# ChanTsune/Portable-Network-Archive

Hardware: AMD Instinct MI355X
Metric: archive-create MiB/s (input bytes/sec), zstd-3, 10000 x 1 MiB enwik-style corpus (higher is better)
Workload: dtype u8

## Files before the change

portable-network-archive_amd/csrc/k_lz_split.hip:

```cpp
#include <type_traits>
#include "lz_common.h"

namespace pna {


#define DPP_ROW_SHL1(v) ((uint32_t)__builtin_amdgcn_update_dpp(0, (int)(v), 0x101, 0xF, 0xF, true))
constexpr uint32_t PK_LEN = 26, PK_OFF = 6, PK_LOW = (1u << PK_LEN) - 1;
__host__ __device__ constexpr uint32_t pkb_of(int strong) { return strong == 2 ? 2u : 3u; }
__device__ __forceinline__ uint32_t pk_make(uint32_t l, uint32_t off, uint32_t bkf) { return (l << PK_LEN) | ((off << PK_OFF) | bkf); }
template <uint32_t S, uint32_t PKB = 3>
__device__ __forceinline__ uint32_t pk_adopt(uint32_t P, uint32_t Pn) {
    constexpr uint32_t BM = PKB == 2 ? 0x3Cu : 0x38u;
    const uint32_t T = Pn + ((S << PK_LEN) - (S << PKB));
    const bool a = (Pn & (BM & ~((S - 1) << PKB))) != 0 && T > (P | PK_LOW);
    return a ? T : P;
}
#define DPP_ROW_SHL2(v) ((uint32_t)__builtin_amdgcn_update_dpp(0, (int)(v), 0x102, 0xF, 0xF, true))
__device__ __forceinline__ uint32_t ffbh_hw(uint32_t x) { uint32_t r; asm("v_ffbh_u32 %0, %1" : "=v"(r) : "v"(x)); return r; }
__device__ __forceinline__ uint32_t back15_field(uint32_t x1, uint32_t x2, uint32_t x3, uint32_t x4) {
    const uint32_t f1 = ffbh_hw(x1), f2 = __builtin_elementwise_add_sat(ffbh_hw(x2), 32u), f3 = __builtin_elementwise_add_sat(ffbh_hw(x3), 64u), f4 = ffbh_hw(x4 | 0xFFu) + 96u;
    uint32_t n, m;
    asm("v_min3_u32 %0, %1, %2, %3" : "=v"(n) : "v"(f2), "v"(f3), "v"(f4));
    asm("v_min_u32 %0, %1, %2" : "=v"(m) : "v"(f1), "v"(n));
    return (m >> 1) & 0x3Cu;
// ... 391 lines not shown
                    l = 16 + first_diff16(y0, y1, y2, y3);
                }
                if (edge) { const uint32_t lim = blk_end - q; l = l < lim ? l : lim; }
                const uint32_t bqj = j ? __builtin_amdgcn_alignbyte(D[0], Dm1, j) : Dm1;
                const uint32_t xk = bqj ^ bc;
                uint32_t bk3 = (uint32_t)__builtin_clz(xk | 0xFFu) & 24u;
                if (STRONG == 1 && xk == 0) { const uint32_t bq2 = j ? __builtin_amdgcn_alignbyte(Dm1, Dm2, j) : Dm2; bk3 = 32u + ((uint32_t)__builtin_clz((bq2 ^ bc2) | 0xFFu) & 24u); }
                if (STRONG == 2) {
                    lds_cu32 *pe = lds_word(WB8 + 8 + ((c8 - 8) & ~3u));
                    const uint32_t e0 = pe[0], e1 = pe[1], p0 = pc[0];
                    const uint32_t bq2 = j ? __builtin_amdgcn_alignbyte(Dm1, Dm2, j) : Dm2, bq3 = j ? __builtin_amdgcn_alignbyte(Dm2, Dm3, j) : Dm3, bq4 = j ? __builtin_amdgcn_alignbyte(Dm3, Dm4, j) : Dm4;
                    bk3 = back15_field(xk, bq2 ^ bc2, bq3 ^ __builtin_amdgcn_alignbit(p0, e1, shc), bq4 ^ __builtin_amdgcn_alignbit(e1, e0, shc));
                }
                Pj = STRONG ? (l >= MIN_MATCH ? pk_make(l, o, bk3) : 0u) : pk_make(l >= MIN_MATCH ? l : 0u, o, bk3);
            }
            P[j] = Pj;
        }
        if (adopt) {
            if (STRONG == 2) {
                uint32_t P8[4];
#pragma unroll
                for (int j = 0; j < 4; j++) P8[j] = DPP_ROW_SHL2(P[j]);
#pragma unroll
                for (int j = 0; j < 4; j++) P[j] = pk_adopt<8, PKB>(P[j], P8[j]);
            }
            if (STRONG) {
                uint32_t P4[4];
#pragma unroll
                for (int j = 0; j < 4; j++) P4[j] = DPP_ROW_SHL1(P[j]);
#pragma unroll
                for (int j = 0; j < 4; j++) P[j] = pk_adopt<4, PKB>(P[j], P4[j]);
            }
            {
                const uint32_t Pn = DPP_ROW_SHL1(P[0]);
                const uint32_t P1[4] = {P[1], P[2], P[3], Pn};
#pragma unroll
                for (int j = 0; j < 4; j++) P[j] = pk_adopt<1, PKB>(P[j], P1[j]);
            }
            {
                const uint32_t Pa = DPP_ROW_SHL1(P[0]), Pb = DPP_ROW_SHL1(P[1]);
                const uint32_t P2[4] = {P[2], P[3], Pa, Pb};
#pragma unroll
                for (int j = 0; j < 4; j++) P[j] = pk_adopt<2, PKB>(P[j], P2[j]);
            }
        }
        if (q0 < t1) {
            if (W3) {
                uint32_t ww[4];
#pragma unroll
                for (int j = 0; j < 4; j++) {
                    const uint32_t l = P[j] >> PK_LEN, lc = l < 5u ? 5u : (l > 36u ? 36u : l);
                    ww[j] = (lc - 5u) | ((P[j] >> (PK_OFF - 5)) & (0xFFFFFu << 5));
                }
                W12 *o = (W12 *)(pb8 + 3 * (size_t)q0);
                __builtin_nontemporal_store(__builtin_amdgcn_perm(ww[1], ww[0], 0x04020100u), &o->x);
                __builtin_nontemporal_store(__builtin_amdgcn_perm(ww[2], ww[1], 0x05040201u), &o->y);
                __builtin_nontemporal_store(__builtin_amdgcn_perm(ww[3], ww[2], 0x06050402u), &o->z);
            } else {
                const uint32_t lmax = (flags & FLAG_LEN36) ? 36u : 63u;
                uint32_t l4[4];
#pragma unroll
                for (int j = 0; j < 4; j++) { const uint32_t l = P[j] >> PK_LEN; l4[j] = l < lmax ? l : lmax; }
                v4u wv;
                wv.x = l4[0] | (P[0] & (0xFFFFFu << PK_OFF)); wv.y = l4[1] | (P[1] & (0xFFFFFu << PK_OFF));
                wv.z = l4[2] | (P[2] & (0xFFFFFu << PK_OFF)); wv.w = l4[3] | (P[3] & (0xFFFFFu << PK_OFF));
                __builtin_nontemporal_store(wv, (v4u *)(pb + q0));
            }
        }
#undef QW
#pragma unroll
        for (int j = 0; j < 4; j++) if (hv[j] && (ins_all || !(j & 1))) atomicMax(&table[hsh[j]], ((q0 + j + 1) << TAG_BITS) | tag[j]);
        __syncthreads();
    }
}

constexpr uint32_t LZP_THREADS = 64;
template <bool CT, int LZD, bool W3>
__global__ __launch_bounds__(LZP_THREADS) __attribute__((amdgpu_waves_per_eu(5, 5)))
void k_lzp(const uint8_t *__restrict__ src, const SegDesc *__restrict__ segs, const uint32_t *__restrict__ blk_seg, uint64_t *__restrict__ seqs, uint8_t *__restrict__ lits,
           BlkInfo *__restrict__ blk, uint4 *__restrict__ ctab, uint32_t flags, uint32_t max_len, const uint32_t *__restrict__ pbuf, uint32_t blk0, uint32_t *__restrict__ hist) {
    constexpr uint32_t RW = 256, TG = 4096;
    static_assert(LZ_G_ZSTD == 4 && LZ_G_DEFLATE == 4 && (1u << BLK_LOG_MIN) % TG == 0 && CAP1 == 32, "k_lzp: regions of 4 groups, tiles of 16 regions");
    __shared__ __attribute__((aligned(16))) uint32_t l32[TG / 4];
    __shared__ uint4 lmask[TG / 64];
    __shared__ uint32_t plut[16];
    uint4 (*rec)[TG / 64] = (uint4 (*)[TG / 64])l32;
    __shared__ uint16_t xlen[16 * 8];
    __shared__ uint32_t shist[192];
    __shared__ uint8_t s_llc[64], s_mlc[128];
    __shared__ uint32_t lstage[264];
    const uint32_t lane = threadIdx.x, w = lane & 15;
    const uint8_t *len8 = (const uint8_t *)l32;
    const uint32_t gb = blk0 + blockIdx.x;
    const SegDesc sd = segs[blk_seg[gb]];
    const uint32_t seg_len = sd.len;
    if ((flags & FLAG_SMALL_ONLY) && seg_len > MID_SEG) return;
    const uint8_t *seg = src + sd.src_off;
    const uint32_t blk_log = sd.blk_log, bsz = 1u << blk_log, SC = seq_cap_of(blk_log);
    const uint32_t *pb = pbuf + ((size_t)(sd.blk_base - blk0) << blk_log);
    const uint8_t *pb8 = (const uint8_t *)pbuf + 3 * ((size_t)(sd.blk_base - blk0) << blk_log);
    auto word_at = [&](uint32_t pos) -> uint32_t {
        if (!W3) return pb[pos];
        const uint32_t x = *(const u32u *)(pb8 + 3 * (size_t)pos) & 0xFFFFFFu, e = x & 31u;
        return (e ? e + 5u : 0u) | ((x >> 5) << 6);
    };
    const uint32_t lazy = flags & F_LAZY;
    const uint32_t wbase = w * RW;
    const uint32_t bs0 = (gb - sd.blk_base) << blk_log, bs1 = seg_len - bs0 < bsz ? seg_len : bs0 + bsz;
    const uint32_t tile0 = bs0 / TG, ntile = bs0 < seg_len ? (bs1 + TG - 1) / TG : tile0;
    const bool lv = lane < 16;
    if (hist) {
        const uint32_t i = lane, m0 = lane, m1 = lane + 64;
        s_llc[i] = (uint8_t)(i < 16 ? i : (i < 24 ? 16 + ((i - 16) >> 1) : (i < 32 ? 20 + ((i - 24) >> 2) : (i < 48 ? 22 + ((i - 32) >> 3) : 24))));
        s_mlc[m0] = (uint8_t)(m0 < 32 ? m0 : (m0 < 40 ? 32 + ((m0 - 32) >> 1) : (m0 < 48 ? 36 + ((m0 - 40) >> 2) : 38 + ((m0 - 48) >> 3))));
        s_mlc[m1] = (uint8_t)(m1 < 96 ? 40 + ((m1 - 64) >> 4) : 42);
    }
    if (lv) {
        uint32_t sel = 0, j = 0;
        for (uint32_t bit = 0; bit < 4; bit++) if ((lane >> bit) & 1) { sel |= bit << (8 * j); j++; }
        plut[lane] = sel;
    }
    const uint64_t lit_below = ((uint64_t)1 << (4 * (lane & 15))) - 1;
    uint32_t next_free = 0, seq_run = 0, lit_run = 0, g_last1 = 1;
    uint32_t lcarry = 0;

    for (uint32_t T = tile0; T < ntile; T++) {
        const uint32_t t0 = T * TG, blk_start = t0 & ~(bsz - 1);
        const uint32_t blk_end = (seg_len - blk_start < bsz) ? seg_len : blk_start + bsz;
        const uint32_t t1 = (blk_end - t0 < TG) ? blk_end : t0 + TG;
        const uint32_t npos = t1 - t0;
        const uint32_t ext_lim = (t1 + LOOKAHEAD < blk_end) ? t1 + LOOKAHEAD : blk_end;
        const uint32_t gblk = sd.blk_base + (t0 >> blk_log);
        const uint32_t ng = (npos + 63) >> 6;
        {
            const uint4 *pt = (const uint4 *)(pb + t0);
            const W12 *pt3 = (const W12 *)(pb8 + 3 * (size_t)t0);
            for (uint32_t wq = 0; wq < 4 && wq * 1024 < npos; wq++) {
                uint4 v[4]; W12 v3[4];
#pragma unroll
                for (uint32_t i = 0; i < 4; i++) { if (W3) v3[i] = pt3[(wq * 4 + i) * 64 + lane]; else v[i] = pt[(wq * 4 + i) * 64 + lane]; }
#pragma unroll
                for (uint32_t i = 0; i < 4; i++) {
                    const uint32_t p = (wq * 4 + i) * RW + lane * 4;
                    uint32_t d;
                    if (W3) {
                        const uint32_t E = (v3[i].x & 31u) | (((v3[i].x >> 24) & 31u) << 8) | (((v3[i].y >> 16) & 31u) << 16) | (((v3[i].z >> 8) & 31u) << 24);
                        const uint32_t nz = ((E + 0x1F1F1F1Fu) >> 5) & 0x01010101u;
                        d = E + nz * 5u;
                    } else d = (v[i].x & 63u) | ((v[i].y & 63u) << 8) | ((v[i].z & 63u) << 16) | ((v[i].w & 63u) << 24);
                    if (npos < TG && p + 4 > npos) d = p >= npos ? 0u : d & (0xFFFFFFFFu >> (8 * (p + 4 - npos)));
                    l32[p >> 2] = d;
                }
            }
        }
        __builtin_amdgcn_wave_barrier();
        if (lane < ng) {
            uint32_t d[17];
#pragma unroll
            for (uint32_t i = 0; i < 4; i++) { const uint4 t = ((const uint4 *)l32)[lane * 4 + i]; d[4 * i] = t.x; d[4 * i + 1] = t.y; d[4 * i + 2] = t.z; d[4 * i + 3] = t.w; }
            d[16] = 0;
            uint32_t em2[2] = {0, 0}, cm2[2] = {0, 0};
#pragma unroll
            for (uint32_t i = 0; i < 16; i++) {
                const uint32_t x = d[i] | 0x80808080u;
                uint32_t e = x - 0x06060606u;
                if (lazy) {
                    e &= x - __builtin_amdgcn_alignbyte(d[i + 1], d[i], 1);
                    if (LZD >= 2) e &= x + 0x01010101u - __builtin_amdgcn_alignbyte(d[i + 1], d[i], 2);
                    if (LZD >= 3) e &= x + 0x02020202u - __builtin_amdgcn_alignbyte(d[i + 1], d[i], 3);
                }
                const uint32_t en = ((((e >> 7) & 0x01010101u) * 0x00204081u) >> 21) & 15u;
                const uint32_t cn = ((((d[i] >> 5) & 0x01010101u) * 0x00204081u) >> 21) & 15u;
                em2[i >> 3] |= en << (4 * (i & 7)); cm2[i >> 3] |= cn << (4 * (i & 7));
            }
            lmask[lane] = make_uint4(em2[0], em2[1], cm2[0], cm2[1]);
        }
        __builtin_amdgcn_wave_barrier();
        if (t0 == blk_start) { next_free = blk_start; seq_run = 0; lit_run = 0; g_last1 = 1; lcarry = 0;
                               if (hist) { for (uint32_t i = lane; i < 192; i += 64) shist[i] = 0; __builtin_amdgcn_wave_barrier(); } }
        const uint32_t c_in = next_free > t0 ? next_free - t0 : 0u;
        uint64_t sel[4], cov[4], cm[4];
        uint32_t el = 0, nx = 0;
        uint32_t em_lo[4], em_hi[4], cm_lo[4], cm_hi[4];
#pragma unroll
        for (int r = 0; r < 4; r++) {
            uint4 m = make_uint4(0, 0, 0, 0);
            if (lv && w * 4 + r < ng) m = lmask[w * 4 + r];
            em_lo[r] = m.x; em_hi[r] = m.y; cm_lo[r] = m.z; cm_hi[r] = m.w;
        }
        {
            uint32_t cur = c_in > wbase ? (c_in - wbase < RW ? c_in - wbase : RW) : 0u;
            uint32_t s32[8], c32[8];
#pragma unroll
            for (int hb = 0; hb < 8; hb++) {
                const uint32_t em32 = (hb & 1) ? em_hi[hb >> 1] : em_lo[hb >> 1], cm32 = (hb & 1) ? cm_hi[hb >> 1] : cm_lo[hb >> 1];
                const uint32_t e0 = cur > 32u * hb ? cur - 32u * hb : 0u;
                uint32_t rem = e0 < 32 ? em32 & (0xFFFFFFFFu << e0) : 0u;
                uint32_t e_last = e0, selr = 0, covr = e0 < 32 ? (1u << e0) - 1 : 0xFFFFFFFFu;
                while (__ballot(rem != 0)) {
                    const bool a = rem != 0;
                    const uint32_t s = a ? (uint32_t)__builtin_ctz(rem) : 0u;
                    const uint32_t ps = wbase + 32u * hb + s;
                    uint32_t L = a ? len8[ps] : 0u;
                    const bool cap = a && ((cm32 >> s) & 1);
                    uint64_t need = __ballot(cap);
                    if (need) {
                        const uint32_t qs = t0 + ps;
                        const uint32_t pwv = cap ? word_at(qs) : 0u;
                        const uint32_t xl = ext_lim - qs < max_len ? ext_lim - qs : max_len;
                        while (need) {
                            const uint32_t k = ctz64(need); need &= need - 1;
                            const uint32_t qk = rdlane(qs, k), ok = rdlane(pwv >> 6, k);
                            const uint32_t Lk = lz_extend_mem(seg, seg_len, qk, qk - ok, rdlane(L, k), rdlane(xl, k), lane);
                            if (lane == k) L = Lk;
                        }
                        if (cap) { xlen[w * 8 + (nx & 7)] = (uint16_t)L; nx++; }
                    }
                    if (a) {
                        const uint32_t e = s + L;
                        const uint32_t me = e < 32 ? (1u << e) - 1 : 0xFFFFFFFFu;
                        selr |= 1u << s; e_last = e;
                        covr |= me & ~((1u << s) - 1);
                        rem &= ~me;
                    }
                }
                s32[hb] = selr; c32[hb] = covr;
                if (selr) el = 32u * hb + e_last;
                cur = 32u * hb + (e_last > 32 ? e_last : 32u);
            }
#pragma unroll
            for (int r = 0; r < 4; r++) {
                sel[r] = (uint64_t)s32[2 * r] | ((uint64_t)s32[2 * r + 1] << 32); cov[r] = (uint64_t)c32[2 * r] | ((uint64_t)c32[2 * r + 1] << 32);
                cm[r] = (uint64_t)cm_lo[r] | ((uint64_t)cm_hi[r] << 32);
            }
        }
        uint32_t pc[4];
        pc[0] = 0;
#pragma unroll
        for (int r = 0; r < 3; r++) pc[r + 1] = pc[r] + (uint32_t)__popcll(sel[r] & cm[r]);

        uint32_t E = c_in, tile_exit;
        {
            const uint32_t wend = el ? wbase + el : 0u;
            uint32_t x = c_in;
#pragma unroll
            for (uint32_t k = 0; k < 16; k++) {
                const uint32_t ek = rdlane(wend, k);
                if (w == k) E = x;
                if (x < k * RW + RW && ek >= x + CUT_MIN) x = ek;
            }
            tile_exit = x;
        }
        uint64_t fsel[4], litm[4];
        uint32_t nselp[5], nlitp[5];
        uint32_t cut_r = 4, cut_b = 0, cut_len = 0, cut_off = 0;
        {
            const uint32_t Ew = E > wbase ? (E - wbase < RW ? E - wbase : RW) : 0u;
            const uint32_t in0 = t1 > t0 + wbase ? t1 - (t0 + wbase) : 0u;
            uint64_t K[4], cv[4];
#pragma unroll
            for (int r = 0; r < 4; r++) {
                const uint32_t e = Ew > 64u * r ? Ew - 64u * r : 0u;
                K[r] = mlow(e < 64 ? e : 64u); fsel[r] = sel[r] & ~K[r]; cv[r] = cov[r];
            }
            if (lv && Ew > 0 && Ew < RW) {
                const uint32_t grp = Ew >> 6, b = Ew & 63;
                uint64_t cg = cov[0], sg = sel[0];
#pragma unroll
                for (int r = 1; r < 4; r++) if (grp == (uint32_t)r) { cg = cov[r]; sg = sel[r]; }
                if (((cg >> b) & 1) && !((sg >> b) & 1)) {
                    uint64_t below = sg & mlow(b);
                    uint32_t g2 = grp;
#pragma unroll
                    for (int r = 2; r >= 0; r--) if (!below && (uint32_t)r < grp && sel[r]) { below = sel[r]; g2 = (uint32_t)r; }
                    const uint32_t s2 = 63 - clz64(below);
                    const uint32_t pw2 = word_at(t0 + wbase + 64 * g2 + s2);
                    uint64_t sc2 = sel[0] & cm[0]; uint32_t pc2 = pc[0];
#pragma unroll
                    for (int r = 1; r < 4; r++) if (g2 == (uint32_t)r) { sc2 = sel[r] & cm[r]; pc2 = pc[r]; }
                    const uint32_t l2 = ((sc2 >> s2) & 1) ? xlen[w * 8 + ((pc2 + (uint32_t)__popcll(sc2 & mlow(s2))) & 7)] : (pw2 & 63u);
                    const uint32_t end2 = 64 * g2 + s2 + l2, rmn = end2 - Ew;
                    if (rmn >= CUT_MIN) {
#pragma unroll
                        for (int r = 0; r < 4; r++) if (grp == (uint32_t)r) fsel[r] |= (uint64_t)1 << b;
                        cut_r = grp; cut_b = b; cut_len = rmn; cut_off = pw2 >> 6;
                    } else {
                        uint32_t fx_s = RW, fx_x = 0;
                        if (end2 < RW) {
                            uint64_t eg = 0, eg1 = 0, cg2 = 0, cg3 = 0;
#pragma unroll
                            for (int r = 0; r < 4; r++) {
                                const uint64_t e64 = (uint64_t)em_lo[r] | ((uint64_t)em_hi[r] << 32);
                                if (grp == (uint32_t)r) { eg = e64; cg2 = cm[r]; }
                                if (grp + 1 == (uint32_t)r) { eg1 = e64; cg3 = cm[r]; }
                            }
                            const uint32_t want = (1u << rmn) - 1u;
                            const uint32_t w8 = (uint32_t)((eg >> b) | (b ? eg1 << (64 - b) : 0)) & want, c8 = (uint32_t)((cg2 >> b) | (b ? cg3 << (64 - b) : 0));
                            if (w8) {
                                const uint32_t ds = (uint32_t)__builtin_ctz(w8), sp = Ew + ds;
                                const uint32_t L = len8[wbase + sp], x = sp + L;
                                if (!((c8 >> ds) & 1) && x < RW && x < in0) {
                                    const uint32_t gx = x >> 6, bx = x & 63;
                                    uint64_t cvx = cov[0], slx = sel[0];
#pragma unroll
                                    for (int r = 1; r < 4; r++) if (gx == (uint32_t)r) { cvx = cov[r]; slx = sel[r]; }
                                    if (!((cvx >> bx) & 1) || ((slx >> bx) & 1)) { fx_s = sp; fx_x = x; }
                                }
                            }
                        }
#pragma unroll
                        for (int r = 0; r < 4; r++) {
                            const uint32_t a0 = Ew > 64u * r ? (Ew - 64u * r < 64 ? Ew - 64u * r : 64u) : 0u;
                            const uint32_t zend = fx_s < RW ? fx_x : end2;
                            const uint32_t z0 = zend > 64u * r ? (zend - 64u * r < 64 ? zend - 64u * r : 64u) : 0u;
                            cv[r] &= ~(mlow(z0) & ~mlow(a0));
                            if (fx_s < RW) {
                                const uint32_t s0 = fx_s > 64u * r ? (fx_s - 64u * r < 64 ? fx_s - 64u * r : 64u) : 0u;
                                cv[r] |= mlow(z0) & ~mlow(s0);
                                fsel[r] &= ~mlow(z0);
                                if ((fx_s >> 6) == (uint32_t)r) fsel[r] |= (uint64_t)1 << (fx_s & 63);
                            }
                        }
                    }
                }
            }
            nselp[0] = 0; nlitp[0] = 0;
#pragma unroll
            for (int r = 0; r < 4; r++) {
                const uint32_t ir = in0 > 64u * r ? in0 - 64u * r : 0u;
                litm[r] = lv ? mlow(ir < 64 ? ir : 64u) & ~(cv[r] | K[r]) : 0;
                if (!lv) fsel[r] = 0;
                nselp[r + 1] = nselp[r] + (uint32_t)__popcll(fsel[r]);
                nlitp[r + 1] = nlitp[r] + (uint32_t)__popcll(litm[r]);
            }
        }
        uint32_t gl = 0, gf = 0;
#pragma unroll
        for (int r = 3; r >= 0; r--) if (!gl && fsel[r]) { const uint32_t sp = 63 - clz64(fsel[r]); gl = 1 + nlitp[r] + (uint32_t)__popcll(litm[r] & mlow(sp)); }
        if (CT) {
#pragma unroll
            for (int r = 0; r < 4; r++) if (!gf && fsel[r]) { const uint32_t sp = ctz64(fsel[r]); gf = 1 + nlitp[r] + (uint32_t)__popcll(litm[r] & mlow(sp)); }
        }
        {
            const uint32_t cnt = nselp[4] | (nlitp[4] << 16);
            const uint32_t incl = row_scan_add(cnt), excl = incl - cnt;
            const uint32_t gabs = gl ? lit_run + (excl >> 16) + gl : 0u;
            const uint32_t gmax = row_scan_max(gabs);
            const uint32_t tot = rdlane(incl, 15);
            const uint32_t seq_base = seq_run + (excl & 0xFFFF), lit_base = lit_run + (excl >> 16);
            const uint32_t gb = DPP_ROW_SHR(gmax, 1);
            const uint32_t glast1_before = gb > g_last1 ? gb : g_last1;
            const uint32_t ga = rdlane(gmax, 15);
            if (CT) {
                constexpr uint32_t CH = TG / TILE, WPC = 16 / CH;
                const uint32_t hrow = (uint32_t)__ballot(gl != 0) & 0xFFFFu;
#pragma unroll
                for (uint32_t h = 0; h < CH; h++) {
                    const uint32_t ex_h = rdlane(excl, h * WPC);
                    const uint32_t hm_h = hrow & (((1u << WPC) - 1) << (h * WPC));
                    uint32_t g_first = lit_run + (tot >> 16);
                    if (hm_h) { const uint32_t j0 = (uint32_t)__builtin_ctz(hm_h); g_first = lit_run + (rdlane(excl, j0) >> 16) + rdlane(gf, j0) - 1; }
                    if (lane == 0) ctab[((size_t)gblk << (blk_log - 11)) + (t0 - blk_start) / TILE + h] = make_uint4(seq_run + (ex_h & 0xFFFF), lit_run + (ex_h >> 16), g_first, 0u);
                }
            }
            g_last1 = ga > g_last1 ? ga : g_last1;
            seq_run += tot & 0xFFFF; lit_run += tot >> 16;
            next_free = t0 + rdlane(tile_exit, 0);
            asm volatile("" ::: "memory");
            if (lv) {
                uint32_t prevl = 0; bool any = false;
#pragma unroll
                for (int r = 0; r < 4; r++) {
                    const uint32_t llbase = any ? nlitp[r] - prevl : lit_base + nlitp[r] - (glast1_before - 1);
                    if (fsel[r]) { const uint32_t sp = 63 - clz64(fsel[r]); prevl = nlitp[r] + (uint32_t)__popcll(litm[r] & mlow(sp)); any = true; }
                    const uint64_t sc = sel[r] & cm[r];
                    const uint32_t cutw = cut_r == (uint32_t)r ? cut_b | (cut_len << 8) : 64u;
                    rec[0][w * 4 + r] = make_uint4((uint32_t)litm[r], (uint32_t)(litm[r] >> 32), lit_base + nlitp[r], seq_base + nselp[r]);
                    rec[1][w * 4 + r] = make_uint4((uint32_t)fsel[r], (uint32_t)(fsel[r] >> 32), (uint32_t)sc, (uint32_t)(sc >> 32));
                    rec[2][w * 4 + r] = make_uint4(llbase, w * 8 + pc[r], cutw, cut_off);
                }
            }
            if (t1 == blk_end && lane == 0) { blk[gblk].nseq = seq_run; blk[gblk].nlit = lit_run; }
        }
        __builtin_amdgcn_wave_barrier();
        uint32_t lw[16];
        if (t0 + TG <= seg_len) {
#pragma unroll
            for (uint32_t wr = 0; wr < 16; wr++) lw[wr] = *(const uint32_t *)(seg + t0 + wr * RW + 4 * lane);
        } else {
#pragma unroll
            for (uint32_t wr = 0; wr < 16; wr++) {
                const uint32_t q = t0 + wr * RW + 4 * lane;
                lw[wr] = 0;
                if (q + 4 <= seg_len) lw[wr] = *(const uint32_t *)(seg + q);
                else { for (uint32_t i = 0; i < 3; i++) if (q + i < seg_len) lw[wr] |= (uint32_t)seg[q + i] << (8 * i); }
            }
        }
        {
            uint64_t *bseq = seqs + (size_t)gblk * SC;
            const uint4 ra = rec[0][lane], rb = rec[1][lane], rc = rec[2][lane];
            const uint64_t lm = (uint64_t)ra.x | ((uint64_t)ra.y << 32), sc = (uint64_t)rb.z | ((uint64_t)rb.w << 32);
            uint64_t rem = lane < ng ? (uint64_t)rb.x | ((uint64_t)rb.y << 32) : 0;
            uint32_t idx = ra.w, prev = 0;
            const uint32_t cut_b2 = rc.z & 0xFFu, cut_l2 = rc.z >> 8;
            bool first = true;
            const uint32_t pg0 = t0 + lane * 64;
            while (rem) {
                uint32_t sq[4], pw[4];
#pragma unroll
                for (int u = 0; u < 4; u++) {
                    sq[u] = rem ? ctz64(rem) : 64u;
                    pw[u] = rem ? word_at(pg0 + sq[u]) : 0u;
                    rem &= rem - 1;
                }
#pragma unroll
                for (int u = 0; u < 4; u++) {
                    const uint32_t s = sq[u];
                    if (s < 64) {
                        uint32_t ml = pw[u] & 63u, of = pw[u] >> 6;
                        if ((sc >> s) & 1) ml = xlen[(rc.y + (uint32_t)__popcll(sc & mlow(s))) & 127];
                        if (cut_b2 == s) { ml = cut_l2; of = rc.w; }
                        const uint32_t lq = (uint32_t)__popcll(lm & mlow(s));
                        const uint32_t ll = first ? rc.x + lq : lq - prev;
                        if (idx < SC) bseq[idx] = seq_pack(ll, ml, of);
                        if (hist) {
                            const uint32_t mb = ml - 3u, of3 = of + 3u;
                            uint32_t *hh = shist;
                            atomicAdd(&hh[ll < 64 ? (uint32_t)s_llc[ll] : 50u - (uint32_t)__builtin_clz(ll)], 1u);
                            atomicAdd(&hh[64 + 31u - (uint32_t)__builtin_clz(of3)], 1u);
                            atomicAdd(&hh[128 + (mb < 128 ? (uint32_t)s_mlc[mb] : 67u - (uint32_t)__builtin_clz(mb))], 1u);
                        }
                        idx++; prev = lq; first = false;
                    }
                }
            }
        }
        if (hist && t1 == blk_end) {
            __builtin_amdgcn_wave_barrier(); asm volatile("" ::: "memory");
            uint32_t *hs = hist + (size_t)blk_seg[gb] * 448u + 256u;
            for (uint32_t i = lane; i < 192; i += 64) { const uint32_t v = shist[i]; if (v) atomicAdd(&hs[i], v); }
        }
        {
            uint8_t *blit = lits + ((size_t)gblk << blk_log);
            const uint32_t sh = 4 * (lane & 15);
            uint8_t *stage8 = (uint8_t *)lstage;
#pragma unroll
            for (uint32_t wq = 0; wq < 4; wq++) {
                if (wq * 1024 >= npos) continue;
                const uint32_t L0 = rec[0][wq * 16].z, L1 = wq < 3 ? rec[0][wq * 16 + 16].z : lit_run;
                const uint32_t A0 = L0 & ~3u;
                if (lane == 0) lstage[0] = lcarry;
                __builtin_amdgcn_wave_barrier(); asm volatile("" ::: "memory");
#pragma unroll
                for (uint32_t i = 0; i < 4; i++) {
                    const uint32_t wr = wq * 4 + i;
                    if (wr * RW >= npos) continue;
                    const uint4 m = rec[0][wr * 4 + (lane >> 4)];
                    const uint32_t wd = lw[wr];
                    const uint64_t lm = (uint64_t)m.x | ((uint64_t)m.y << 32);
                    const uint32_t nib = (uint32_t)(lm >> sh) & 15u;
                    const uint32_t pk = __builtin_amdgcn_perm(wd, wd, plut[nib]), cnt = (uint32_t)__popc(nib);
                    uint8_t *o = stage8 + (m.z + (uint32_t)__popcll(lm & lit_below) - A0);
                    if (cnt > 0) o[0] = (uint8_t)pk;
                    if (cnt > 1) o[1] = (uint8_t)(pk >> 8);
                    if (cnt > 2) o[2] = (uint8_t)(pk >> 16);
                    if (cnt > 3) o[3] = (uint8_t)(pk >> 24);
                }
                __builtin_amdgcn_wave_barrier(); asm volatile("" ::: "memory");
                const uint32_t nfull = (L1 - A0) >> 2;
                uint32_t *g32 = (uint32_t *)(blit + A0);
                for (uint32_t j = lane; j < nfull; j += 64) g32[j] = lstage[j];
                lcarry = uni(lstage[nfull]);
                __builtin_amdgcn_wave_barrier(); asm volatile("" ::: "memory");
            }
            if (t1 == blk_end) {
                const uint32_t rem = lit_run & 3u;
                if (lane < rem) blit[(lit_run & ~3u) + lane] = (uint8_t)(lcarry >> (8 * lane));
            }
        }
        __builtin_amdgcn_wave_barrier();
        asm volatile("" ::: "memory");
    }
}

template <bool CT, int STRONG, uint32_t GLOG, uint32_t WLOG, bool FARP = !CT, bool TAB3 = false>
static void launch_split_g(const uint8_t *src, const SegDesc *segs, uint32_t nseg, uint64_t *seqs, uint8_t *lits, BlkInfo *blk, uint4 *ctab,
                           uint32_t flags, uint32_t max_off, uint32_t max_len, hipStream_t st, uint32_t *pbuf, uint32_t blk0, hipEvent_t ev_match, uint32_t *gtab, const LzParseGrid *pg) {
    constexpr uint32_t LT = GLOG ? LzGeo<WLOG>::L_TABLE : LzGeo<WLOG, TAB3>::L_TOTAL;
    static const hipError_t attr_set = hipFuncSetAttribute((const void *)k_lzm<CT, STRONG, GLOG, WLOG, FARP, TAB3>, hipFuncAttributeMaxDynamicSharedMemorySize, (int)LzGeo<WLOG, TAB3>::L_TOTAL);
    (void)attr_set;
    constexpr bool W3 = GLOG == 0;
    if (!(flags & FLAG_ALL_SMALL)) hipLaunchKernelGGL((k_lzm<CT, STRONG, GLOG, WLOG, FARP, TAB3>), dim3(nseg), dim3(LZ_THREADS), LT, st, src, segs, flags, max_off, pbuf, blk0, gtab);
    if (flags & FLAG_TIER1) hipLaunchKernelGGL((k_lzms<STRONG, W3>), dim3(nseg), dim3(64), lzms_lds(SMALL_SEG), st, src, segs, flags, pbuf, blk0, 0u, SMALL_SEG);
    if (flags & FLAG_TIER2) { const uint32_t mx = 8192u + 4096u * ((flags >> FLAG_T2_SHIFT) & 3u);
                              hipLaunchKernelGGL((k_lzms<STRONG, W3>), dim3(nseg), dim3(64), lzms_lds(mx), st, src, segs, flags, pbuf, blk0, SMALL_SEG, mx); }
    if (ev_match) (void)hipEventRecord(ev_match, st);
    if (!pg || pg->nb == 0) return;
    if (flags & FLAG_LAZY3) hipLaunchKernelGGL((k_lzp<CT, 3, W3>), dim3(pg->nb), dim3(LZP_THREADS), 0, st, src, pg->segs_all, pg->blk_seg, seqs, lits, blk, ctab, flags, max_len, pbuf, blk0, pg->hist);
    else if (flags & FLAG_LAZY2) hipLaunchKernelGGL((k_lzp<CT, 2, W3>), dim3(pg->nb), dim3(LZP_THREADS), 0, st, src, pg->segs_all, pg->blk_seg, seqs, lits, blk, ctab, flags, max_len, pbuf, blk0, pg->hist);
    else hipLaunchKernelGGL((k_lzp<CT, 1, W3>), dim3(pg->nb), dim3(LZP_THREADS), 0, st, src, pg->segs_all, pg->blk_seg, seqs, lits, blk, ctab, flags, max_len, pbuf, blk0, pg->hist);
}
void launch_lz_split(const uint8_t *src, const SegDesc *segs, uint32_t nseg, uint64_t *seqs, uint8_t *lits, BlkInfo *blk, uint4 *ctab,
                     uint32_t flags, uint32_t max_off, uint32_t max_len, hipStream_t st, uint32_t *pbuf, uint32_t blk0, hipEvent_t ev_match, uint32_t *gtab, const LzParseGrid *pg) {
// ... 48 lines not shown
```

Baseline: 145,600.

## Parallelize greedy match selection across all 64 lanes with speculative group resync

The greedy parse over each 256-byte region is no longer walked serially by 16 lanes across four 64-bit groups. All 64 lanes now walk one 64-position group each in parallel, starting at the group boundary, then repair speculation by re-walking from the predecessor's actual end until the walk synchronizes with an already selected match. Extended lengths are packed per lane into two 16-bit slots instead of a shared ring, and prefix scans are widened to span 64 lanes. This is meant to remove the serial dependency and idle lanes in match selection, at the cost of redundant re-walks when groups don't resynchronize. It also caps extended matches at two per group.

Measured after the change: 146,200, median of 6. About the same (+0.4%).

```diff
diff --git a/portable-network-archive_amd/csrc/k_lz_split.hip b/portable-network-archive_amd/csrc/k_lz_split.hip
--- a/portable-network-archive_amd/csrc/k_lz_split.hip
+++ b/portable-network-archive_amd/csrc/k_lz_split.hip
@@ -497,14 +497,14 @@
     constexpr uint32_t RW = 256, TG = 4096;
     static_assert(LZ_G_ZSTD == 4 && LZ_G_DEFLATE == 4 && (1u << BLK_LOG_MIN) % TG == 0 && CAP1 == 32, "k_lzp: regions of 4 groups, tiles of 16 regions");
     __shared__ __attribute__((aligned(16))) uint32_t l32[TG / 4];
-    __shared__ uint4 lmask[TG / 64];
+    __shared__ uint4 gsc[TG / 64];
     __shared__ uint32_t plut[16];
     uint4 (*rec)[TG / 64] = (uint4 (*)[TG / 64])l32;
-    __shared__ uint16_t xlen[16 * 8];
+    __shared__ uint32_t xlen[TG / 64];
     __shared__ uint32_t shist[192];
     __shared__ uint8_t s_llc[64], s_mlc[128];
     __shared__ uint32_t lstage[264];
-    const uint32_t lane = threadIdx.x, w = lane & 15;
+    const uint32_t lane = threadIdx.x, w = lane >> 2, rq = lane & 3;
     const uint8_t *len8 = (const uint8_t *)l32;
     const uint32_t gb = blk0 + blockIdx.x;
     const SegDesc sd = segs[blk_seg[gb]];
@@ -520,17 +520,16 @@
         return (e ? e + 5u : 0u) | ((x >> 5) << 6);
     };
     const uint32_t lazy = flags & F_LAZY;
-    const uint32_t wbase = w * RW;
+    const uint32_t wbase = w * RW, gb64 = 64 * rq, gbase = 64 * lane;
     const uint32_t bs0 = (gb - sd.blk_base) << blk_log, bs1 = seg_len - bs0 < bsz ? seg_len : bs0 + bsz;
     const uint32_t tile0 = bs0 / TG, ntile = bs0 < seg_len ? (bs1 + TG - 1) / TG : tile0;
-    const bool lv = lane < 16;
     if (hist) {
         const uint32_t i = lane, m0 = lane, m1 = lane + 64;
         s_llc[i] = (uint8_t)(i < 16 ? i : (i < 24 ? 16 + ((i - 16) >> 1) : (i < 32 ? 20 + ((i - 24) >> 2) : (i < 48 ? 22 + ((i - 32) >> 3) : 24))));
         s_mlc[m0] = (uint8_t)(m0 < 32 ? m0 : (m0 < 40 ? 32 + ((m0 - 32) >> 1) : (m0 < 48 ? 36 + ((m0 - 40) >> 2) : 38 + ((m0 - 48) >> 3))));
         s_mlc[m1] = (uint8_t)(m1 < 96 ? 40 + ((m1 - 64) >> 4) : 42);
     }
-    if (lv) {
+    if (lane < 16) {
         uint32_t sel = 0, j = 0;
         for (uint32_t bit = 0; bit < 4; bit++) if ((lane >> bit) & 1) { sel |= bit << (8 * j); j++; }
         plut[lane] = sel;
@@ -569,6 +568,7 @@
             }
         }
         __builtin_amdgcn_wave_barrier();
+        uint64_t em = 0, cm = 0;
         if (lane < ng) {
             uint32_t d[17];
 #pragma unroll
@@ -588,193 +588,192 @@
                 const uint32_t cn = ((((d[i] >> 5) & 0x01010101u) * 0x00204081u) >> 21) & 15u;
                 em2[i >> 3] |= en << (4 * (i & 7)); cm2[i >> 3] |= cn << (4 * (i & 7));
             }
-            lmask[lane] = make_uint4(em2[0], em2[1], cm2[0], cm2[1]);
-        }
-        __builtin_amdgcn_wave_barrier();
+            em = (uint64_t)em2[0] | ((uint64_t)em2[1] << 32); cm = (uint64_t)cm2[0] | ((uint64_t)cm2[1] << 32);
+        }
         if (t0 == blk_start) { next_free = blk_start; seq_run = 0; lit_run = 0; g_last1 = 1; lcarry = 0;
                                if (hist) { for (uint32_t i = lane; i < 192; i += 64) shist[i] = 0; __builtin_amdgcn_wave_barrier(); } }
         const uint32_t c_in = next_free > t0 ? next_free - t0 : 0u;
-        uint64_t sel[4], cov[4], cm[4];
-        uint32_t el = 0, nx = 0;
-        uint32_t em_lo[4], em_hi[4], cm_lo[4], cm_hi[4];
-#pragma unroll
-        for (int r = 0; r < 4; r++) {
-            uint4 m = make_uint4(0, 0, 0, 0);
-            if (lv && w * 4 + r < ng) m = lmask[w * 4 + r];
-            em_lo[r] = m.x; em_hi[r] = m.y; cm_lo[r] = m.z; cm_hi[r] = m.w;
-        }
+        const uint32_t rent = c_in > wbase ? (c_in - wbase < RW ? c_in - wbase : RW) : 0u;
+        uint64_t sel = 0, cov;
+        uint32_t ext, le = 0, xl2 = 0;
+        auto walk_len = [&](bool a, uint32_t s) -> uint32_t {
+            uint32_t L = a ? len8[gbase + s] : 0u;
+            const bool cap = a && ((cm >> s) & 1);
+            uint64_t need = __ballot(cap);
+            if (need) {
+                const uint32_t qs = t0 + gbase + s;
+                const uint32_t pwv = cap ? word_at(qs) : 0u;
+                const uint32_t xl = ext_lim - qs < max_len ? ext_lim - qs : max_len;
+                while (need) {
+                    const uint32_t k = ctz64(need); need &= need - 1;
+                    const uint32_t qk = rdlane(qs, k), ok = rdlane(pwv >> 6, k);
+                    const uint32_t Lk = lz_extend_mem(seg, seg_len, qk, qk - ok, rdlane(L, k), rdlane(xl, k), lane);
+                    if (lane == k) L = Lk;
+                }
+            }
+            return L;
+        };
+        const uint32_t ent = rent > gb64 ? rent : gb64;
         {
-            uint32_t cur = c_in > wbase ? (c_in - wbase < RW ? c_in - wbase : RW) : 0u;
-            uint32_t s32[8], c32[8];
-#pragma unroll
-            for (int hb = 0; hb < 8; hb++) {
-                const uint32_t em32 = (hb & 1) ? em_hi[hb >> 1] : em_lo[hb >> 1], cm32 = (hb & 1) ? cm_hi[hb >> 1] : cm_lo[hb >> 1];
-                const uint32_t e0 = cur > 32u * hb ? cur - 32u * hb : 0u;
-                uint32_t rem = e0 < 32 ? em32 & (0xFFFFFFFFu << e0) : 0u;
-                uint32_t e_last = e0, selr = 0, covr = e0 < 32 ? (1u << e0) - 1 : 0xFFFFFFFFu;
-                while (__ballot(rem != 0)) {
-                    const bool a = rem != 0;
-                    const uint32_t s = a ? (uint32_t)__builtin_ctz(rem) : 0u;
-                    const uint32_t ps = wbase + 32u * hb + s;
-                    uint32_t L = a ? len8[ps] : 0u;
-                    const bool cap = a && ((cm32 >> s) & 1);
-                    uint64_t need = __ballot(cap);
-                    if (need) {
-                        const uint32_t qs = t0 + ps;
-                        const uint32_t pwv = cap ? word_at(qs) : 0u;
-                        const uint32_t xl = ext_lim - qs < max_len ? ext_lim - qs : max_len;
-                        while (need) {
-                            const uint32_t k = ctz64(need); need &= need - 1;
-                            const uint32_t qk = rdlane(qs, k), ok = rdlane(pwv >> 6, k);
-                            const uint32_t Lk = lz_extend_mem(seg, seg_len, qk, qk - ok, rdlane(L, k), rdlane(xl, k), lane);
-                            if (lane == k) L = Lk;
-                        }
-                        if (cap) { xlen[w * 8 + (nx & 7)] = (uint16_t)L; nx++; }
-                    }
-                    if (a) {
-                        const uint32_t e = s + L;
-                        const uint32_t me = e < 32 ? (1u << e) - 1 : 0xFFFFFFFFu;
-                        selr |= 1u << s; e_last = e;
-                        covr |= me & ~((1u << s) - 1);
-                        rem &= ~me;
-                    }
-                }
-                s32[hb] = selr; c32[hb] = covr;
-                if (selr) el = 32u * hb + e_last;
-                cur = 32u * hb + (e_last > 32 ? e_last : 32u);
-            }
-#pragma unroll
-            for (int r = 0; r < 4; r++) {
-                sel[r] = (uint64_t)s32[2 * r] | ((uint64_t)s32[2 * r + 1] << 32); cov[r] = (uint64_t)c32[2 * r] | ((uint64_t)c32[2 * r + 1] << 32);
-                cm[r] = (uint64_t)cm_lo[r] | ((uint64_t)cm_hi[r] << 32);
-            }
-        }
-        uint32_t pc[4];
-        pc[0] = 0;
-#pragma unroll
-        for (int r = 0; r < 3; r++) pc[r + 1] = pc[r] + (uint32_t)__popcll(sel[r] & cm[r]);
+            const uint32_t e0 = ent - gb64;
+            cov = mlow(e0);
+            uint64_t rem = em & ~cov;
+            uint32_t nx = 0;
+            while (__ballot(rem != 0)) {
+                const bool a = rem != 0;
+                const uint32_t s = a ? ctz64(rem) : 0u;
+                const uint32_t L = walk_len(a, s);
+                if (a) {
+                    const uint32_t e = s + L;
+                    const uint64_t me = mlow(e);
+                    if ((cm >> s) & 1) { xl2 |= L << (16 * nx); nx++; }
+                    sel |= (uint64_t)1 << s; cov |= me & ~mlow(s); rem &= ~me;
+                    le = gb64 + e;
+                }
+            }
+            ext = ent > le ? ent : le; ext = ext > gb64 + 64 ? ext : gb64 + 64;
+        }
+#pragma unroll
+        for (uint32_t k = 1; k < 4; k++) {
+            const uint32_t te = DPP_ROW_SHR(ext, 1);
+            const bool fix = rq == k && te > ent;
+            if (!__ballot(fix)) continue;
+            bool act = fix, synced = false;
+            uint32_t c = te, ss = 0, rnx = 0, rxl = 0, rle = 0;
+            uint64_t rsel = 0, rcov = mlow(te - gb64);
+            while (__ballot(act)) {
+                uint32_t s = 0;
+                if (act) {
+                    const uint32_t e0 = c - gb64;
+                    const uint64_t rr = e0 < 64 ? em & ~mlow(e0) : 0;
+                    if (!rr) act = false;
+                    else { s = ctz64(rr); if ((sel >> s) & 1) { synced = true; ss = s; act = false; } }
+                }
+                const uint32_t L = walk_len(act, s);
+                if (act) {
+                    const uint32_t e = s + L;
+                    if ((cm >> s) & 1) { rxl |= L << (16 * rnx); rnx++; }
+                    rsel |= (uint64_t)1 << s; rcov |= mlow(e) & ~mlow(s);
+                    c = gb64 + e; rle = c;
+                }
+            }
+            if (fix) {
+                if (synced) {
+                    const uint64_t keep = ~mlow(ss);
+                    const uint32_t r0 = (uint32_t)__popcll(sel & cm & mlow(ss));
+                    xl2 = (uint32_t)(rxl | (((uint64_t)xl2 >> (16 * r0)) << (16 * rnx)));
+                    sel = rsel | (sel & keep); cov = rcov | (cov & keep);
+                } else {
+                    sel = rsel; cov = rcov; le = rle; xl2 = rxl;
+                    ext = c > gb64 + 64 ? c : gb64 + 64;
+                }
+            }
+        }
+        gsc[lane] = make_uint4((uint32_t)sel, (uint32_t)(sel >> 32), (uint32_t)cov, (uint32_t)(cov >> 32));
+        xlen[lane] = xl2;
+        uint32_t lsq = sel ? gb64 + 64 - clz64(sel) : 0u, leq = le;
+        {
+            const uint32_t s1 = DPP_ROW_SHR(lsq, 1), e1 = DPP_ROW_SHR(leq, 1);
+            if (rq >= 1) { lsq = lsq > s1 ? lsq : s1; leq = leq > e1 ? leq : e1; }
+            const uint32_t s2 = DPP_ROW_SHR(lsq, 2), e2 = DPP_ROW_SHR(leq, 2);
+            if (rq >= 2) { lsq = lsq > s2 ? lsq : s2; leq = leq > e2 ? leq : e2; }
+        }
+        const uint32_t pls0 = DPP_ROW_SHR(lsq, 1), ple0 = DPP_ROW_SHR(leq, 1);
+        const uint32_t pls = rq >= 1 ? pls0 : 0u, ple = rq >= 1 ? ple0 : 0u;
+        const uint64_t em1n = (uint64_t)DPP_ROW_SHL1((uint32_t)em) | ((uint64_t)DPP_ROW_SHL1((uint32_t)(em >> 32)) << 32);
+        const uint64_t cm1n = (uint64_t)DPP_ROW_SHL1((uint32_t)cm) | ((uint64_t)DPP_ROW_SHL1((uint32_t)(cm >> 32)) << 32);
+        const uint64_t em1 = rq < 3 ? em1n : 0, cm1 = rq < 3 ? cm1n : 0;
 
         uint32_t E = c_in, tile_exit;
         {
-            const uint32_t wend = el ? wbase + el : 0u;
+            const uint32_t wend = leq ? wbase + leq : 0u;
             uint32_t x = c_in;
 #pragma unroll
             for (uint32_t k = 0; k < 16; k++) {
-                const uint32_t ek = rdlane(wend, k);
+                const uint32_t ek = rdlane(wend, 4 * k + 3);
                 if (w == k) E = x;
                 if (x < k * RW + RW && ek >= x + CUT_MIN) x = ek;
             }
             tile_exit = x;
         }
-        uint64_t fsel[4], litm[4];
-        uint32_t nselp[5], nlitp[5];
-        uint32_t cut_r = 4, cut_b = 0, cut_len = 0, cut_off = 0;
-        {
-            const uint32_t Ew = E > wbase ? (E - wbase < RW ? E - wbase : RW) : 0u;
-            const uint32_t in0 = t1 > t0 + wbase ? t1 - (t0 + wbase) : 0u;
-            uint64_t K[4], cv[4];
-#pragma unroll
-            for (int r = 0; r < 4; r++) {
-                const uint32_t e = Ew > 64u * r ? Ew - 64u * r : 0u;
-                K[r] = mlow(e < 64 ? e : 64u); fsel[r] = sel[r] & ~K[r]; cv[r] = cov[r];
-            }
-            if (lv && Ew > 0 && Ew < RW) {
-                const uint32_t grp = Ew >> 6, b = Ew & 63;
-                uint64_t cg = cov[0], sg = sel[0];
-#pragma unroll
-                for (int r = 1; r < 4; r++) if (grp == (uint32_t)r) { cg = cov[r]; sg = sel[r]; }
-                if (((cg >> b) & 1) && !((sg >> b) & 1)) {
-                    uint64_t below = sg & mlow(b);
-                    uint32_t g2 = grp;
-#pragma unroll
-                    for (int r = 2; r >= 0; r--) if (!below && (uint32_t)r < grp && sel[r]) { below = sel[r]; g2 = (uint32_t)r; }
+        const uint32_t Ew = E > wbase ? (E - wbase < RW ? E - wbase : RW) : 0u;
+        const uint32_t in0 = t1 > t0 + wbase ? t1 - (t0 + wbase) : 0u;
+        const uint64_t K = mlow(Ew > gb64 ? Ew - gb64 : 0u);
+        uint64_t fsel = sel & ~K, cv = cov;
+        uint32_t cutw = 64u, cut_off = 0, fxp = 0;
+        if (Ew > 0 && Ew < RW && (Ew >> 6) == rq) {
+            const uint32_t b = Ew & 63;
+            if (((cov >> b) & 1) && !((sel >> b) & 1)) {
+                const uint64_t below = sel & mlow(b);
+                uint32_t p2, end2;
+                if (below) {
                     const uint32_t s2 = 63 - clz64(below);
-                    const uint32_t pw2 = word_at(t0 + wbase + 64 * g2 + s2);
-                    uint64_t sc2 = sel[0] & cm[0]; uint32_t pc2 = pc[0];
-#pragma unroll
-                    for (int r = 1; r < 4; r++) if (g2 == (uint32_t)r) { sc2 = sel[r] & cm[r]; pc2 = pc[r]; }
-                    const uint32_t l2 = ((sc2 >> s2) & 1) ? xlen[w * 8 + ((pc2 + (uint32_t)__popcll(sc2 & mlow(s2))) & 7)] : (pw2 & 63u);
-                    const uint32_t end2 = 64 * g2 + s2 + l2, rmn = end2 - Ew;
-                    if (rmn >= CUT_MIN) {
-#pragma unroll
-                        for (int r = 0; r < 4; r++) if (grp == (uint32_t)r) fsel[r] |= (uint64_t)1 << b;
-                        cut_r = grp; cut_b = b; cut_len = rmn; cut_off = pw2 >> 6;
-                    } else {
-                        uint32_t fx_s = RW, fx_x = 0;
-                        if (end2 < RW) {
-                            uint64_t eg = 0, eg1 = 0, cg2 = 0, cg3 = 0;
-#pragma unroll
-                            for (int r = 0; r < 4; r++) {
-                                const uint64_t e64 = (uint64_t)em_lo[r] | ((uint64_t)em_hi[r] << 32);
-                                if (grp == (uint32_t)r) { eg = e64; cg2 = cm[r]; }
-                                if (grp + 1 == (uint32_t)r) { eg1 = e64; cg3 = cm[r]; }
-                            }
-                            const uint32_t want = (1u << rmn) - 1u;
-                            const uint32_t w8 = (uint32_t)((eg >> b) | (b ? eg1 << (64 - b) : 0)) & want, c8 = (uint32_t)((cg2 >> b) | (b ? cg3 << (64 - b) : 0));
-                            if (w8) {
-                                const uint32_t ds = (uint32_t)__builtin_ctz(w8), sp = Ew + ds;
-                                const uint32_t L = len8[wbase + sp], x = sp + L;
-                                if (!((c8 >> ds) & 1) && x < RW && x < in0) {
-                                    const uint32_t gx = x >> 6, bx = x & 63;
-                                    uint64_t cvx = cov[0], slx = sel[0];
-#pragma unroll
-                                    for (int r = 1; r < 4; r++) if (gx == (uint32_t)r) { cvx = cov[r]; slx = sel[r]; }
-                                    if (!((cvx >> bx) & 1) || ((slx >> bx) & 1)) { fx_s = sp; fx_x = x; }
-                                }
-                            }
-                        }
-#pragma unroll
-                        for (int r = 0; r < 4; r++) {
-                            const uint32_t a0 = Ew > 64u * r ? (Ew - 64u * r < 64 ? Ew - 64u * r : 64u) : 0u;
-                            const uint32_t zend = fx_s < RW ? fx_x : end2;
-                            const uint32_t z0 = zend > 64u * r ? (zend - 64u * r < 64 ? zend - 64u * r : 64u) : 0u;
-                            cv[r] &= ~(mlow(z0) & ~mlow(a0));
-                            if (fx_s < RW) {
-                                const uint32_t s0 = fx_s > 64u * r ? (fx_s - 64u * r < 64 ? fx_s - 64u * r : 64u) : 0u;
-                                cv[r] |= mlow(z0) & ~mlow(s0);
-                                fsel[r] &= ~mlow(z0);
-                                if ((fx_s >> 6) == (uint32_t)r) fsel[r] |= (uint64_t)1 << (fx_s & 63);
+                    p2 = gb64 + s2;
+                    const uint64_t sc = sel & cm;
+                    end2 = ((sc >> s2) & 1) ? p2 + ((xl2 >> (16 * (uint32_t)__popcll(sc & mlow(s2)))) & 0xFFFFu) : 0u;
+                } else { p2 = pls - 1; end2 = ple; }
+                const uint32_t pw2 = word_at(t0 + wbase + p2);
+                if (!end2) end2 = p2 + (pw2 & 63u);
+                const uint32_t rmn = end2 - Ew;
+                if (rmn >= CUT_MIN) {
+                    fsel |= (uint64_t)1 << b;
+                    cutw = b | (rmn << 8); cut_off = pw2 >> 6;
+                } else {
+                    uint32_t fx_s = RW, fx_x = 0;
+                    if (end2 < RW) {
+                        const uint32_t want = (1u << rmn) - 1u;
+                        const uint32_t w8 = (uint32_t)((em >> b) | (b ? em1 << (64 - b) : 0)) & want, c8 = (uint32_t)((cm >> b) | (b ? cm1 << (64 - b) : 0));
+                        if (w8) {
+                            const uint32_t ds = (uint32_t)__builtin_ctz(w8), sp = Ew + ds;
+                            const uint32_t L = len8[wbase + sp], x = sp + L;
+                            if (!((c8 >> ds) & 1) && x < RW && x < in0) {
+                                const uint4 gx = gsc[w * 4 + (x >> 6)];
+                                const uint32_t bx = x & 31, cvx = (x & 32) ? gx.w : gx.z, slx = (x & 32) ? gx.y : gx.x;
+                                if (!((cvx >> bx) & 1) || ((slx >> bx) & 1)) { fx_s = sp; fx_x = x; }
                             }
                         }
                     }
-                }
-            }
-            nselp[0] = 0; nlitp[0] = 0;
-#pragma unroll
-            for (int r = 0; r < 4; r++) {
-                const uint32_t ir = in0 > 64u * r ? in0 - 64u * r : 0u;
-                litm[r] = lv ? mlow(ir < 64 ? ir : 64u) & ~(cv[r] | K[r]) : 0;
-                if (!lv) fsel[r] = 0;
-                nselp[r + 1] = nselp[r] + (uint32_t)__popcll(fsel[r]);
-                nlitp[r + 1] = nlitp[r] + (uint32_t)__popcll(litm[r]);
-            }
-        }
-        uint32_t gl = 0, gf = 0;
-#pragma unroll
-        for (int r = 3; r >= 0; r--) if (!gl && fsel[r]) { const uint32_t sp = 63 - clz64(fsel[r]); gl = 1 + nlitp[r] + (uint32_t)__popcll(litm[r] & mlow(sp)); }
-        if (CT) {
-#pragma unroll
-            for (int r = 0; r < 4; r++) if (!gf && fsel[r]) { const uint32_t sp = ctz64(fsel[r]); gf = 1 + nlitp[r] + (uint32_t)__popcll(litm[r] & mlow(sp)); }
-        }
+                    fxp = (fx_s < RW ? fx_x : end2) | (fx_s < RW ? (fx_s + 1) << 16 : 0u);
+                }
+            }
+        }
+        fxp = (uint32_t)__shfl((int)fxp, (int)(w * 4 + ((Ew >> 6) & 3)));
+        if (fxp) {
+            const uint32_t zend = fxp & 0xFFFFu, z0 = zend > gb64 ? zend - gb64 : 0u;
+            cv &= ~(mlow(z0) & ~K);
+            if (fxp >> 16) {
+                const uint32_t fx_s = (fxp >> 16) - 1, s0 = fx_s > gb64 ? fx_s - gb64 : 0u;
+                cv |= mlow(z0) & ~mlow(s0);
+                fsel &= ~mlow(z0);
+                if ((fx_s >> 6) == rq) fsel |= (uint64_t)1 << (fx_s & 63);
+            }
+        }
+        const uint64_t litm = mlow(in0 > gb64 ? in0 - gb64 : 0u) & ~(cv | K);
         {
-            const uint32_t cnt = nselp[4] | (nlitp[4] << 16);
-            const uint32_t incl = row_scan_add(cnt), excl = incl - cnt;
-            const uint32_t gabs = gl ? lit_run + (excl >> 16) + gl : 0u;
-            const uint32_t gmax = row_scan_max(gabs);
-            const uint32_t tot = rdlane(incl, 15);
+            const uint32_t cnt = (uint32_t)__popcll(fsel) | ((uint32_t)__popcll(litm) << 16);
+            const uint32_t rinc = row_scan_add(cnt);
+            const uint32_t r0 = rdlane(rinc, 15), r01 = r0 + rdlane(rinc, 31), r012 = r01 + rdlane(rinc, 47);
+            const uint32_t incl = rinc + (lane < 16 ? 0u : lane < 32 ? r0 : lane < 48 ? r01 : r012), excl = incl - cnt;
+            const uint32_t tot = rdlane(incl, 63);
             const uint32_t seq_base = seq_run + (excl & 0xFFFF), lit_base = lit_run + (excl >> 16);
-            const uint32_t gb = DPP_ROW_SHR(gmax, 1);
-            const uint32_t glast1_before = gb > g_last1 ? gb : g_last1;
-            const uint32_t ga = rdlane(gmax, 15);
+            const uint32_t gabs = fsel ? lit_base + 1 + (uint32_t)__popcll(litm & mlow(63 - clz64(fsel))) : 0u;
+            const uint32_t rmax = row_scan_max(gabs);
+            const uint32_t m0 = rdlane(rmax, 15), m1 = rdlane(rmax, 31), m2 = rdlane(rmax, 47), m3 = rdlane(rmax, 63);
+            const uint32_t m01 = m0 > m1 ? m0 : m1, m012 = m01 > m2 ? m01 : m2;
+            const uint32_t rpre = lane < 16 ? 0u : lane < 32 ? m0 : lane < 48 ? m01 : m012;
+            uint32_t glast1_before = DPP_ROW_SHR(rmax, 1);
+            glast1_before = glast1_before > rpre ? glast1_before : rpre; glast1_before = glast1_before > g_last1 ? glast1_before : g_last1;
+            const uint32_t ga = m012 > m3 ? m012 : m3;
             if (CT) {
-                constexpr uint32_t CH = TG / TILE, WPC = 16 / CH;
-                const uint32_t hrow = (uint32_t)__ballot(gl != 0) & 0xFFFFu;
+                constexpr uint32_t CH = TG / TILE, GPC = 64 / CH;
+                const uint64_t hm = __ballot(fsel != 0);
+                const uint32_t gf = fsel ? lit_base + (uint32_t)__popcll(litm & mlow(ctz64(fsel))) : 0u;
 #pragma unroll
                 for (uint32_t h = 0; h < CH; h++) {
-                    const uint32_t ex_h = rdlane(excl, h * WPC);
-                    const uint32_t hm_h = hrow & (((1u << WPC) - 1) << (h * WPC));
+                    const uint32_t ex_h = rdlane(excl, h * GPC);
+                    const uint64_t hm_h = (hm >> (h * GPC)) & mlow(GPC);
                     uint32_t g_first = lit_run + (tot >> 16);
-                    if (hm_h) { const uint32_t j0 = (uint32_t)__builtin_ctz(hm_h); g_first = lit_run + (rdlane(excl, j0) >> 16) + rdlane(gf, j0) - 1; }
+                    if (hm_h) g_first = rdlane(gf, h * GPC + ctz64(hm_h));
                     if (lane == 0) ctab[((size_t)gblk << (blk_log - 11)) + (t0 - blk_start) / TILE + h] = make_uint4(seq_run + (ex_h & 0xFFFF), lit_run + (ex_h >> 16), g_first, 0u);
                 }
             }
@@ -782,19 +781,10 @@
             seq_run += tot & 0xFFFF; lit_run += tot >> 16;
             next_free = t0 + rdlane(tile_exit, 0);
             asm volatile("" ::: "memory");
-            if (lv) {
-                uint32_t prevl = 0; bool any = false;
-#pragma unroll
-                for (int r = 0; r < 4; r++) {
-                    const uint32_t llbase = any ? nlitp[r] - prevl : lit_base + nlitp[r] - (glast1_before - 1);
-                    if (fsel[r]) { const uint32_t sp = 63 - clz64(fsel[r]); prevl = nlitp[r] + (uint32_t)__popcll(litm[r] & mlow(sp)); any = true; }
-                    const uint64_t sc = sel[r] & cm[r];
-                    const uint32_t cutw = cut_r == (uint32_t)r ? cut_b | (cut_len << 8) : 64u;
-                    rec[0][w * 4 + r] = make_uint4((uint32_t)litm[r], (uint32_t)(litm[r] >> 32), lit_base + nlitp[r], seq_base + nselp[r]);
-                    rec[1][w * 4 + r] = make_uint4((uint32_t)fsel[r], (uint32_t)(fsel[r] >> 32), (uint32_t)sc, (uint32_t)(sc >> 32));
-                    rec[2][w * 4 + r] = make_uint4(llbase, w * 8 + pc[r], cutw, cut_off);
-                }
-            }
+            const uint64_t sc = sel & cm;
+            rec[0][lane] = make_uint4((uint32_t)litm, (uint32_t)(litm >> 32), lit_base, seq_base);
+            rec[1][lane] = make_uint4((uint32_t)fsel, (uint32_t)(fsel >> 32), (uint32_t)sc, (uint32_t)(sc >> 32));
+            rec[2][lane] = make_uint4(lit_base - (glast1_before - 1), 0u, cutw, cut_off);
             if (t1 == blk_end && lane == 0) { blk[gblk].nseq = seq_run; blk[gblk].nlit = lit_run; }
         }
         __builtin_amdgcn_wave_barrier();
@@ -833,7 +823,7 @@
                     const uint32_t s = sq[u];
                     if (s < 64) {
                         uint32_t ml = pw[u] & 63u, of = pw[u] >> 6;
-                        if ((sc >> s) & 1) ml = xlen[(rc.y + (uint32_t)__popcll(sc & mlow(s))) & 127];
+                        if ((sc >> s) & 1) ml = (xlen[lane] >> (16 * (uint32_t)__popcll(sc & mlow(s)))) & 0xFFFFu;
                         if (cut_b2 == s) { ml = cut_l2; of = rc.w; }
                         const uint32_t lq = (uint32_t)__popcll(lm & mlow(s));
                         const uint32_t ll = first ? rc.x + lq : lq - prev;
```
